# NirajNair/vector-indexer

Hardware: AMD Instinct MI355X
Metric: QPS at recall@10>=0.95 (IVF search, SIFT1M-shaped) (higher is better)
Workload: dtype f32; 1 GPU; IVF search N=1000000 D=128 nlist=4096 nprobe=32 k=10 nq/step=10000 (BASELINE configs[1]); nprobe=32, index_centroids=4094, parallelism=1 GPU

## Files before the change

vector-indexer_amd/csrc/range_select.hip:

```cpp
#include <hip/hip_runtime.h>

#include <algorithm>
#include <cmath>
#include <cstdio>
#include <vector>

#include "select.hpp"
#include "select_device.hpp"

namespace vi {

namespace {

constexpr uint64_t kMaxRangeKeys = 1ull << 27;
constexpr uint32_t kMinRowLog = 11;

struct RangeArgs {
  SelectCommon c;
  uint32_t q0, m, P;
  float radius2;
  ListProbes lp;
  uint32_t *bound;
  uint64_t *keys;
  uint32_t logL;
  uint32_t *counts;
  uint32_t *overflow;
};

__device__ __attribute__((noinline)) float exact_dist_fn(uint32_t form, const float *qrow, const uint32_t *qbytes, uint32_t qn_int,
                                                         const uint4 *x, uint32_t dim, bool live) {
  float d = INFINITY;
  if (live) {
    if (form == 3u) d = exact_pair_u8_int(qbytes, qn_int, x, dim);
    else if (form == 2u) d = exact_pair_u8(qrow, x, dim);
    else if (form == 1u) d = exact_pair_bf16(qrow, x, dim);
    else d = exact_pair<kWave>(qrow, (const float4 *)x, dim);
  }
  return d;
}

template <bool EMIT, bool FILT>
__global__ void __launch_bounds__(256, 4) range_select_kernel(RangeArgs a) {
  __shared__ uint32_t s_pick[4][kPickCap], s_lcache[4][kCacheG];
  __shared__ float4 s_tcache[4][kCacheG];
  __shared__ __attribute__((aligned(16))) uint32_t s_qbytes[4][64];
  extern __shared__ __attribute__((aligned(16))) float s_qrows[];
  const int lane = threadIdx.x & (kWave - 1), wave = threadIdx.x >> 6;
  if (blockIdx.x * 4 + wave >= a.m) return;
  const uint32_t q = a.q0 + blockIdx.x * 4 + wave;
  const SelectCommon &c = a.c;
  uint32_t *pick = s_pick[wave], *qbytes = s_qbytes[wave];
  float *qlds = s_qrows + (size_t)wave * c.dim;
  const ProbeRegs pr = load_probe_regs(a.lp, c.gq, q, a.P, lane);
  const GroupRecords gr{c, a.lp.qoff[q], a.lp.qtot[q], s_tcache[wave], s_lcache[wave]};
  const uint64_t below = (1ull << lane) - 1ull;
  const QueryFrame f = query_frame<EMIT>(c, q, lane, qlds, qbytes);
  float thr = INFINITY;
  if (a.radius2 < 1.0e37f) {
    const float w = ((float)(c.dim >> 6) + 9.0f) * 6.1e-8f * (fabsf(a.radius2) + f.qn);
    thr = rank_threshold(c, f, (a.radius2 - f.qn) + w);
  }
  const uint32_t form = c.u8_nat ? (f.q_bytes ? 3u : 2u) : (c.hi_nat ? 1u : 0u);
  const uint4 *xbase = c.u8_nat ? c.u8_nat : (c.hi_nat ? c.hi_nat : (const uint4 *)c.blocks);
  const uint32_t xmult = c.u8_nat ? c.dq / 4u : (c.hi_nat ? c.dq / 2u : c.dq);
  uint64_t *row = EMIT ? a.keys + ((size_t)(q - a.q0) << a.logL) : nullptr;
  const uint32_t cap = EMIT ? 1u << a.logL : 0u;
  uint32_t npick = 0, n_exact = 0, n_scanned = 0, n_sub = 0, cursor = 0;
  auto exact_emit = [&](bool live, uint32_t r, uint32_t pos) {
    const uint32_t fb = (uint32_t)__shfl((int)pr.fb, (int)r);
    const uint32_t g = (uint32_t)__shfl((int)pr.g, (int)r);
    const uint32_t len = (uint32_t)__shfl((int)pr.len, (int)r);
    live = live && pos < len;
    const uint32_t p = live ? pos : 0u;
    if constexpr (FILT) live = live && ((c.allow[fb + p / kWave] >> (p % kWave)) & 1ull) != 0ull;
    n_exact += (uint32_t)__popcll(__ballot(live));
    const float d = exact_dist_fn(form, qlds, qbytes, f.qn_int, xbase + ((size_t)(fb + p / kWave) * xmult) * kWave + (p % kWave), c.dim, live);
    const bool hit = live && d <= a.radius2;
    const uint64_t m = __ballot(hit);
    if (hit) {
      const uint32_t at = cursor + (uint32_t)__popcll(m & below);
      if (at < cap) row[at] = pack_key(d, (g << kPosBits) | pos);
    }
    cursor += (uint32_t)__popcll(m);
  };
  auto drain = [&]() { drain_pick(c, pick, npick, lane, exact_emit); };
  gr.fill(lane);
  for (uint32_t gb = 0; gb < gr.G; gb += kWave) {
    const uint32_t gidx = gb + lane;
    const bool live = gidx < gr.G;
    uint32_t r, seg, hh;
    gr.group_place(gidx, live, r, seg, hh);
    scan_pair_records(c, pr, lane, live && !(gr.group_values(gidx, live).x > thr), r, seg, hh, n_scanned,
                      [&](bool ok, float v, uint32_t, uint32_t rr, uint32_t sub, uint32_t h2) {
                        const bool want = ok && !(v > thr);
                        if constexpr (EMIT) push_sub(pick, npick, n_sub, lane, want, rr, sub, h2, drain);
                        else n_sub += (uint32_t)__popcll(__ballot(want));
                      });
  }
  if constexpr (EMIT) {
    drain();
    if (lane == 0) {
      a.counts[q] = min(cursor, cap);
      if (cursor > cap) atomicOr(a.overflow, 1u);
    }
    if (c.dbg && lane == 0 && (q & c.dbg_mask) == 0u) {
      atomicAdd(&c.dbg[kStatSelExact], (unsigned long long)n_exact);
      atomicAdd(&c.dbg[kStatSelScanned], (unsigned long long)n_scanned);
      atomicAdd(&c.dbg[kStatSelSubBlocks], (unsigned long long)n_sub);
    }
  } else {
    if (lane == 0) a.bound[q] = 16u * n_sub;
  }
}

struct RangeOutArgs {
  const uint64_t *keys;
  uint32_t logL, q0, m, P;
  const uint32_t *counts, *probes, *gorder, *first_block;
  const uint64_t *lims, *ext_ids;
  float *D;
  int64_t *I;
  uint64_t *tie, *slots;
};

__global__ void __launch_bounds__(256) range_output_kernel(RangeOutArgs a) {
  __shared__ uint32_t s_fb[4][kWave];
  const uint32_t lane = threadIdx.x & (kWave - 1), wave = threadIdx.x >> 6;
  if (blockIdx.x * 4 + wave >= a.m) return;
  const uint32_t q = a.q0 + blockIdx.x * 4 + wave;
  if (lane < a.P) {
    const uint32_t l = a.probes[(size_t)q * a.P + lane], g = a.gorder[(size_t)q * a.P + lane];
    if (l != kNoPos && g < kWave) s_fb[wave][g] = a.first_block[l];
  }
  wave_lds_sync();
  const uint64_t *row = a.keys + ((size_t)(q - a.q0) << a.logL);
  const uint64_t at = a.lims[q];
  const uint32_t n = a.counts[q];
  for (uint32_t i = lane; i < n; i += kWave) {
    const uint64_t key = row[i];
    const uint32_t t = (uint32_t)key, g = t >> kPosBits, pos = t & kPosMask;
    const uint64_t gslot = (uint64_t)s_fb[wave][g & 63u] * kWave + pos;
    a.D[at + i] = sortable_f32((uint32_t)(key >> 32));
    a.I[at + i] = (int64_t)a.ext_ids[gslot];
    a.tie[at + i] = ((uint64_t)g << 32) | pos;
    a.slots[at + i] = gslot;
  }
}

}

vi_status launch_range_select(SearchBatch &b, float radius2, const SelectFrame &f, RangeResult *res) {
  const DeviceIndex &ix = b.ix;
  const EngineKnobs &kn = b.kn;
  SearchWorkspace &ws = b.ws();
  const uint64_t nq = b.nq;
  hipStream_t st = b.st();
  VI_TRY(ws.range_bound.reserve(nq + 1));
  VI_TRY(ws.counts.reserve(nq));
  RangeArgs a{list_select_common(b, f), 0u, (uint32_t)nq, b.P, radius2, list_probes(b), ws.range_bound.p, nullptr, 0u, ws.counts.p,
              ws.range_bound.p + nq};
  if (b.flt) a.c.allow = b.flt->allow.p;
  unsigned long long *dbg = a.c.dbg;
  const size_t qsm = 4ull * ix.dim * sizeof(float);
  hipEvent_t ev[5] = {nullptr, nullptr, nullptr, nullptr, nullptr};
  struct EventGuard { hipEvent_t *e; ~EventGuard() { for (int i = 0; i < 5; ++i) if (e[i]) (void)hipEventDestroy(e[i]); } } guard{ev};
  float ms_step[4] = {0.0f, 0.0f, 0.0f, 0.0f};
  auto mark = [&](int i) -> vi_status {
    if (!kn.stats_print) return VI_OK;
    if (!ev[i]) VI_HIP(hipEventCreate(&ev[i]));
    VI_HIP(hipEventRecord(ev[i], st));
    return VI_OK;
  };
  auto lap = [&](int step, int from, int to) {
    float ms = 0.0f;
    if (kn.stats_print && hipEventElapsedTime(&ms, ev[from], ev[to]) == hipSuccess) ms_step[step] += ms;
  };
  a.c.dbg = nullptr;
  VI_HIP(hipMemsetAsync(ws.range_bound.p + nq, 0, sizeof(uint32_t), st));
  VI_TRY(mark(0));
  hipLaunchKernelGGL((range_select_kernel<false, false>), dim3((uint32_t)((nq + 3) / 4)), dim3(256), qsm, st, a);
  VI_HIP(hipGetLastError());
  VI_TRY(mark(1));
  std::vector<uint32_t> h_bound(nq);
  VI_HIP(hipMemcpyAsync(h_bound.data(), ws.range_bound.p, nq * sizeof(uint32_t), hipMemcpyDeviceToHost, st));
  VI_HIP(hipStreamSynchronize(st));
  lap(0, 0, 1);
  a.c.dbg = dbg;
  uint64_t q0 = 0;
  while (q0 < nq) {
    uint32_t logL = kMinRowLog;
    while ((1ull << logL) < h_bound[q0]) ++logL;
    if ((1ull << logL) > kMaxRangeKeys) return fail(VI_ERR_INVALID_INPUT, "a query's radius admits more candidates than the key scratch holds");
    uint64_t m = 1;
    while (q0 + m < nq) {
      uint32_t lg = logL;
      while ((1ull << lg) < h_bound[q0 + m]) ++lg;
      if ((m + 1) << lg > kMaxRangeKeys) break;
      logL = lg;
      ++m;
    }
    const uint64_t L = 1ull << logL;
    VI_TRY(ws.sort_keys.reserve(m * L));
    VI_TRY(mark(0));
    VI_HIP(hipMemsetAsync(ws.sort_keys.p, 0xFF, m * L * sizeof(uint64_t), st));
    a.q0 = (uint32_t)q0; a.m = (uint32_t)m; a.keys = ws.sort_keys.p; a.logL = logL;
    const dim3 grid((uint32_t)((m + 3) / 4));
    if (b.flt) hipLaunchKernelGGL((range_select_kernel<true, true>), grid, dim3(256), qsm, st, a);
    else hipLaunchKernelGGL((range_select_kernel<true, false>), grid, dim3(256), qsm, st, a);
    VI_HIP(hipGetLastError());
    VI_TRY(mark(1));
    VI_TRY(sort_rows_u64(ws.sort_keys.p, m, logL, st));
    VI_TRY(mark(2));
    VI_TRY(range_result_place(res, q0, m, ws.counts.p + q0, st));
    RangeOutArgs o{ws.sort_keys.p, logL, (uint32_t)q0, (uint32_t)m, b.P, ws.counts.p, ws.probes.p, ws.gorder.p, ix.list_first_block.p,
                   res->lims.p, ix.ext_ids.p, res->D.p, res->I.p, res->tie.p, res->slots.p};
    hipLaunchKernelGGL(range_output_kernel, grid, dim3(256), 0, st, o);
    VI_HIP(hipGetLastError());
    VI_TRY(mark(3));
    if (kn.stats_print) {
      VI_HIP(hipStreamSynchronize(st));
      lap(1, 0, 1); lap(2, 1, 2); lap(3, 2, 3);
    }
    q0 += m;
  }
  uint32_t overflow = 0;
  VI_HIP(hipMemcpyAsync(&overflow, ws.range_bound.p + nq, sizeof(uint32_t), hipMemcpyDeviceToHost, st));
  VI_HIP(hipStreamSynchronize(st));
  if (kn.stats_print) {
    uint64_t bound_total = 0;
    for (uint32_t b : h_bound) bound_total += b;
    fprintf(stderr, "range select ms: bound pass %.4f, evaluation %.4f, sort %.4f, placing + output %.4f; hits %llu of a bound of %llu\n",
            ms_step[0], ms_step[1], ms_step[2], ms_step[3], (unsigned long long)res->total, (unsigned long long)bound_total);
  }
  if (overflow) return fail(VI_ERR_OTHER, "radius select: a query found more hits than its bound pass counted");
  return VI_OK;
}

}
```

vector-indexer_amd/csrc/select.hip:

```cpp
#include "select.hpp"

#include <hip/hip_runtime.h>

#include <cmath>

#include "select_device.hpp"
#include "wave_select.hpp"

namespace vi {
namespace {

template <class Top>
__device__ __attribute__((noinline)) Top offer_bulk_fn(Top s, float dist, uint32_t pos, int K) {
  s.offer_bulk(dist, pos, K);
  return s;
}

template <class Top>
__device__ __attribute__((noinline)) Top exact_batch_fn(Top sel, const float *qrow, const float4 *xv, uint32_t dim, bool live,
                                                        uint32_t key, int K) {
  float d = INFINITY;
  if (live) d = exact_pair<kWave>(qrow, xv, dim);
  sel.offer_bulk(d, live ? key : kNoPos, K);
  return sel;
}

template <class Top>
__device__ __attribute__((noinline)) Top exact_batch_u8_fn(Top sel, const float *qrow, const uint4 *xb, uint32_t dim, bool live, uint32_t key,
                                                           int K) {
  float d = INFINITY;
  if (live) d = exact_pair_u8(qrow, xb, dim);
  sel.offer_bulk(d, live ? key : kNoPos, K);
  return sel;
}

template <class Top>
__device__ __attribute__((noinline)) Top exact_batch_u8_int_fn(Top sel, const uint32_t *qb, uint32_t qn, const uint4 *xb, uint32_t dim, bool live,
                                                               uint32_t key, int K) {
  float d = INFINITY;
  if (live) d = exact_pair_u8_int(qb, qn, xb, dim);
  sel.offer_bulk(d, live ? key : kNoPos, K);
  return sel;
}

template <class Top>
__device__ __attribute__((noinline)) Top exact_batch_row_fn(Top sel, const float *qrow, const float4 *xr, uint32_t dim, bool live,
                                                            uint32_t key, int K) {
  float d = INFINITY;
  if (live) d = exact_pair<1>(qrow, xr, dim);
  sel.offer_bulk(d, live ? key : kNoPos, K);
  return sel;
}

constexpr uint32_t kStageFloats = 2048;
template <class Top>
__device__ __attribute__((noinline)) Top exact_batch_rows_staged_fn(Top sel, const float *qrow, const float4 *rows, uint32_t nrows, uint32_t dim,
                                                                    uint32_t cnt, uint32_t pos, int K, float *stage) {
  const uint32_t lane = threadIdx.x & 63u, r0 = lane >> 2, piece = (lane & 3u) ^ ((lane >> 3) & 3u);
  const uint32_t nquad = dim >> 2, nch = nquad >> 2;
  const VI_AS_LDS vf4 *xq = (const VI_AS_LDS vf4 *)(const VI_AS_LDS float *)qrow;
  const uint32_t sbase = (uint32_t)(size_t)(VI_AS_LDS float *)stage;
  const float4 *src[4];
#pragma unroll
  for (uint32_t j = 0; j < 4; ++j)
    src[j] = rows + (size_t)min((uint32_t)__shfl((int)pos, (int)min(r0 + 16u * j, cnt - 1u)), nrows - 1u) * nquad + piece;
  auto issue = [&](uint32_t c) {
#pragma unroll
    for (uint32_t j = 0; j < 4; ++j) glds16_at(src[j] + 4u * c, sbase + (c & 1u) * 4096u + j * 1024u);
  };
  asm volatile("s_waitcnt vmcnt(0)" ::: "memory");
  issue(0u);
  if (nch > 1u) issue(1u);
  const uint32_t swz = (lane >> 1) & 3u;
  float acc = 0.0f;
#pragma unroll 1
  for (uint32_t c = 0; c < nch; ++c) {
    if (c + 1u < nch) asm volatile("s_waitcnt vmcnt(4)" ::: "memory");
    else asm volatile("s_waitcnt vmcnt(0)" ::: "memory");
    const VI_AS_LDS vf4 *rd = (const VI_AS_LDS vf4 *)((const VI_AS_LDS float *)stage + (c & 1u) * 1024u + lane * 16u);
    const vf4 x0 = rd[0u ^ swz], x1 = rd[1u ^ swz], x2 = rd[2u ^ swz], x3 = rd[3u ^ swz];
    const vf4 q0 = xq[4u * c], q1 = xq[4u * c + 1u], q2 = xq[4u * c + 2u], q3 = xq[4u * c + 3u];
#define VI_PK_QUAD(QQ, XX)                                                         \
  {                                                                                \
    const vf2 ta = pk_sub_f32(QQ.xy, XX.xy), tb = pk_sub_f32(QQ.zw, XX.zw);        \
    const vf2 sa = ta * ta, sb = tb * tb;                                          \
    acc = acc + sa.x; acc = acc + sa.y; acc = acc + sb.x; acc = acc + sb.y;        \
  }
    VI_PK_QUAD(q0, x0) VI_PK_QUAD(q1, x1) VI_PK_QUAD(q2, x2) VI_PK_QUAD(q3, x3)
#undef VI_PK_QUAD
    if (c + 2u < nch) {
      asm volatile("s_waitcnt lgkmcnt(0)" ::: "memory");
      issue(c + 2u);
    }
  }
  const bool live = lane < cnt && pos < nrows;
  sel.offer_bulk(live ? acc : INFINITY, live ? pos : kNoPos, K);
  return sel;
}

template <class Top>
__device__ __attribute__((noinline)) Top exact_batch_bf16_fn(Top sel, const float *qrow, const uint4 *xh, uint32_t dim, bool live,
                                                             uint32_t key, int K) {
  float d = INFINITY;
  if (live) d = exact_pair_bf16(qrow, xh, dim);
  sel.offer_bulk(d, live ? key : kNoPos, K);
  return sel;
}


template <class Top, bool FILT = false>
__device__ __forceinline__ void select_body(const SelectCommon &c, uint32_t q, size_t gbase, uint32_t G, uint32_t P,
                                            const ProbeRegs &pr, uint32_t K, int lane, uint32_t *pick, float4 *tcache,
                                            uint32_t *lcache, float *qlds, Top &sel, uint32_t *qbytes = nullptr) {
  const uint64_t below = (1ull << lane) - 1ull;
  const QueryFrame f = query_frame<true>(c, q, lane, qlds, qbytes);
  uint32_t npick = 0, n_exact = 0, n_scanned = 0, n_full = 0, n_sub = 0;
  Top s1;
  float thr = INFINITY;
  sel.init();
  const float *qrow = qlds;
  auto exact_offer = [&](bool live, uint32_t r, uint32_t pos) {
    const uint32_t fb = (uint32_t)__shfl((int)pr.fb, (int)r);
    const uint32_t g = (uint32_t)__shfl((int)pr.g, (int)r);
    const uint32_t len = (uint32_t)__shfl((int)pr.len, (int)r);
    live = live && pos < len && !(c.xmode & 1u);
    if constexpr (FILT) {
      const uint32_t p = live ? pos : 0u;
      live = live && ((c.allow[fb + p / kWave] >> (p % kWave)) & 1ull) != 0ull;
    }
    n_exact += (uint32_t)__popcll(__ballot(live));
    if (c.u8_nat && f.q_bytes)
      sel = exact_batch_u8_int_fn(sel, qbytes, f.qn_int, c.u8_nat + ((size_t)(fb + (live ? pos : 0u) / kWave) * (c.dq / 4)) * kWave + (pos % kWave),
                                  c.dim, live, (g << kPosBits) | pos, (int)K);
    else if (c.u8_nat)
      sel = exact_batch_u8_fn(sel, qrow, c.u8_nat + ((size_t)(fb + (live ? pos : 0u) / kWave) * (c.dq / 4)) * kWave + (pos % kWave), c.dim,
                              live, (g << kPosBits) | pos, (int)K);
    else if (c.hi_nat)
      sel = exact_batch_bf16_fn(sel, qrow, c.hi_nat + ((size_t)(fb + (live ? pos : 0u) / kWave) * (c.dq / 2)) * kWave + (pos % kWave),
                                c.dim, live, (g << kPosBits) | pos, (int)K);
    else
      sel = exact_batch_fn(sel, qrow, c.blocks + ((size_t)(fb + (live ? pos : 0u) / kWave) * c.dq) * kWave + (pos % kWave),
                           c.dim, live, (g << kPosBits) | pos, (int)K);
  };
  auto drain = [&]() { drain_pick(c, pick, npick, lane, exact_offer); };
  auto scan_groups = [&](bool want, uint32_t r, uint32_t seg, uint32_t hh, int mode) {
    scan_pair_records(c, pr, lane, want, r, seg, hh, n_scanned, [&](bool ok, float v, uint32_t j, uint32_t rr, uint32_t sub, uint32_t h2) {
      if (mode == 0) s1 = offer_bulk_fn(s1, ok ? v : INFINITY, ok ? j : kNoPos, (int)K);
      else push_sub(pick, npick, n_sub, lane, ok && !(v > thr), rr, sub, h2, drain);
    });
  };

  unsigned long long tk = c.dbg ? __builtin_amdgcn_s_memtime() : 0ull, tks[6] = {0, 0, 0, 0, 0, 0};
  auto lap = [&](int i) {
    if (c.dbg) {
      const unsigned long long now = __builtin_amdgcn_s_memtime();
      tks[i] += now - tk;
      tk = now;
    }
  };
  const GroupRecords gr{c, gbase, G, tcache, lcache};
  gr.fill(lane);
  lap(0);
  bool any_full = false;
  {
    s1.init();
    float U = INFINITY;
    if (K <= 64u) {
      float lm = INFINITY;
      for (uint32_t gb = 0; gb < G; gb += kWave) {
        const uint32_t gidx = gb + lane;
        lm = fminf(lm, gr.group_values(gidx, gidx < G).x);
      }
      uint64_t kk = pack_key(lm, (uint32_t)lane);
      wave_sort_u64(kk, lane);
      U = sortable_f32((uint32_t)(readlane_u64(kk, (int)K - 1) >> 32));
    }
    uint32_t ncand = 0;
    bool overflow = !(U < INFINITY);
    if (!overflow) {
      for (uint32_t gb = 0; gb < G && !overflow; gb += kWave) {
        const uint32_t gidx = gb + lane;
        const bool live = gidx < G;
        const float4 T = gr.group_values(gidx, live);
        const float tv[4] = {T.x, T.y, T.z, T.w};
#pragma unroll
        for (uint32_t j = 0; j < 4; ++j) {
          const bool pass = live && !(tv[j] > U);
          const uint64_t m = __ballot(pass);
          if (!m) continue;
          const uint32_t cnt = (uint32_t)__popcll(m);
          if (ncand + cnt > kPickCap / 2u) { overflow = true; break; }
          if (pass) {
            const uint32_t at = ncand + (uint32_t)__popcll(m & below);
            pick[2u * at] = __float_as_uint(tv[j]);
            pick[2u * at + 1u] = 4u * gidx + j;
          }
          ncand += cnt;
        }
      }
      wave_lds_sync();
    }
    if (!overflow) {
      for (uint32_t c0 = 0; c0 < ncand; c0 += kWave) {
        const bool live = c0 + lane < ncand;
        const float v = live ? __uint_as_float(pick[2u * (c0 + lane)]) : INFINITY;
        s1 = offer_bulk_fn(s1, v, live ? pick[2u * (c0 + lane) + 1u] : kNoPos, (int)K);
      }
      wave_lds_sync();
    } else {
      s1.init();
      for (uint32_t gb = 0; gb < G; gb += kWave) {
        const uint32_t gidx = gb + lane;
        const bool live = gidx < G;
        s1 = offer_bulk_fn(s1, gr.group_values(gidx, live).x, live ? 4u * gidx : kNoPos, (int)K);
      }
      for (uint32_t gb = 0; gb < G; gb += kWave) {
        const uint32_t gidx = gb + lane;
        const bool live = gidx < G;
        const float4 T = gr.group_values(gidx, live);
        s1 = offer_bulk_fn(s1, T.y, live ? 4u * gidx + 1u : kNoPos, (int)K);
        s1 = offer_bulk_fn(s1, T.z, live ? 4u * gidx + 2u : kNoPos, (int)K);
        s1 = offer_bulk_fn(s1, T.w, live ? 4u * gidx + 3u : kNoPos, (int)K);
      }
    }
    thr = rank_threshold(c, f, s1.kth((int)K));
    for (uint32_t gb = 0; gb < G; gb += kWave) {
      const uint32_t gidx = gb + lane;
      const float4 T = gr.group_values(gidx, gidx < G);
      any_full = any_full || __ballot(gidx < G && T.w <= thr) != 0ull;
    }
  }
  lap(1);
  if (any_full && !f.distrust && !(c.xmode & 4u)) {
    {
      bool keep[2] = {false, false};
#pragma unroll
      for (int e = 0; e < Top::kEntries; ++e) {
        const uint32_t key = s1.ent_p(e);
        const bool mine = key != kNoPos && (uint32_t)(64 * e + lane) < K;
        keep[e] = mine && !(gr.group_values(mine ? (key >> 2) : 0u, true).w <= thr);
      }
      s1.rebuild(keep[0], keep[1], (int)K);
    }
    for (uint32_t gb = 0; gb < G; gb += kWave) {
      const uint32_t gidx = gb + lane;
      const bool live = gidx < G;
      uint32_t r, seg, hh;
      gr.group_place(gidx, live, r, seg, hh);
      scan_groups(live && gr.group_values(gidx, live).w <= thr, r, seg, hh, 0);
    }
    thr = fminf(thr, rank_threshold(c, f, s1.kth((int)K)));
  }
  lap(2);
  for (uint32_t gb = 0; gb < G; gb += kWave) {
    const uint32_t gidx = gb + lane;
    const bool live = gidx < G;
    uint32_t r, seg, hh;
    gr.group_place(gidx, live, r, seg, hh);
    const float4 T = gr.group_values(gidx, live);
    n_full += (uint32_t)__popcll(__ballot(live && T.w <= thr));
    scan_groups(live && !(T.x > thr) && !(c.xmode & 2u), r, seg, hh, 1);
  }
  lap(3);
  drain();
  lap(4);
  if (c.dbg && lane == 0 && (q & c.dbg_mask) == 0u) {
#pragma unroll
    for (int i = 0; i < 5; ++i) atomicAdd(&c.dbg[kStatClocks + i], tks[i]);
    atomicAdd(&c.dbg[kStatSelExact], (unsigned long long)n_exact);
    atomicAdd(&c.dbg[kStatSelScanned], (unsigned long long)n_scanned);
    atomicAdd(&c.dbg[kStatSelQueriesFull], (unsigned long long)(any_full ? 1u : 0u));
    atomicAdd(&c.dbg[kStatSelFullGroups], (unsigned long long)n_full);
    atomicAdd(&c.dbg[kStatSelSubBlocks], (unsigned long long)n_sub);
  }
}

struct SelectArgs {
  SelectCommon c;
  uint32_t nq, P, k;
  ListProbes lp;
  const uint64_t *ext_ids;
  float *D;
  int64_t *I;
  uint64_t *tie, *slots;
  uint32_t *counts;
};

template <class Top, bool FILT = false>
__global__ void __launch_bounds__(256, 4) select_kernel(SelectArgs a) {
  __shared__ uint32_t s_pick[4][kPickCap], s_lcache[4][kCacheG];
  __shared__ float4 s_tcache[4][kCacheG];
  __shared__ __attribute__((aligned(16))) uint32_t s_qbytes[4][64];
  extern __shared__ __attribute__((aligned(16))) float s_qrows[];
  const int lane = threadIdx.x & (kWave - 1), wave = threadIdx.x >> 6;
  const uint32_t q = blockIdx.x * 4 + wave;
  if (q >= a.nq) return;
  uint32_t mylist;
  const ProbeRegs pr = load_probe_regs(a.lp, a.c.gq, q, a.P, lane, &mylist);
  Top sel;
  select_body<Top, FILT>(a.c, q, a.lp.qoff[q], a.lp.qtot[q], a.P, pr, a.k, lane, s_pick[wave], s_tcache[wave],
                   s_lcache[wave], s_qrows + (size_t)wave * a.c.dim, sel, s_qbytes[wave]);
  uint32_t found = 0;
  const uint32_t inv = (uint32_t)__builtin_amdgcn_ds_permute((int)(4u * (mylist != kNoPos ? pr.g : (uint32_t)lane)), lane);
#pragma unroll
  for (int e = 0; e < Top::kEntries; ++e) {
    const uint32_t key = sel.ent_p(e), idx = 64u * (uint32_t)e + (uint32_t)lane;
    const uint32_t g = key >> kPosBits, pos = key & kPosMask;
    const uint32_t r = (uint32_t)__shfl((int)inv, (int)(g & 63u));
    const bool have = idx < a.k && key != kNoPos;
    found += (uint32_t)__popcll(__ballot(have));
    const uint32_t fbk = (uint32_t)__shfl((int)pr.fb, (int)r);
    if (idx < a.k) {
      const size_t o = (size_t)q * a.k + idx;
      if (have) {
        const uint64_t gslot = (uint64_t)fbk * kWave + pos;
        a.D[o] = sel.ent_d(e);
        a.I[o] = (int64_t)a.ext_ids[gslot];
        if (a.tie) a.tie[o] = ((uint64_t)g << 32) | pos;
        if (a.slots) a.slots[o] = gslot;
      } else {
        a.D[o] = INFINITY;
        a.I[o] = -1;
        if (a.tie) a.tie[o] = ~0ull;
        if (a.slots) a.slots[o] = ~0ull;
      }
    }
  }
  if (a.counts && lane == 0) a.counts[q] = found;
}

struct CoarseSelectArgs {
  SelectCommon c;
  uint32_t nq, P, nlists, segb, recs;
  const uint32_t *list_shard, *list_len;
  uint32_t *probes, *gorder, *cnt;
  const float4 *cent_rows;
  uint32_t list_segb0;
  uint32_t *rel, *qtot;
  uint32_t staged;
  uint32_t *pair_rank;
};

__device__ __forceinline__ void write_probe_row(const CoarseSelectArgs &a, uint32_t q, int lane, uint32_t mylist, uint32_t found,
                                                bool lane_order) {
  const uint32_t g = lane_order ? (uint32_t)lane : probe_candidate_order(lane, found, mylist, a.list_shard);
  if ((uint32_t)lane < a.P) {
    a.probes[(size_t)q * a.P + lane] = mylist;
    a.gorder[(size_t)q * a.P + lane] = g;
    if (mylist != kNoPos && a.list_len[mylist] > 0) {
      const uint32_t before = atomicAdd(&a.cnt[subbin_index(mylist, q & (kSubBins - 1), a.nlists)], 1u);
      if (a.pair_rank) a.pair_rank[(size_t)q * a.P + lane] = before;
    }
  }
  uint32_t ng = 0;
  if (mylist != kNoPos) {
    uint32_t sb;
    ng = 2u * list_segments(a.list_len[mylist], a.list_segb0, &sb);
  }
  const uint32_t ig = wave_incl_scan_u32(ng);
  if ((uint32_t)lane < a.P) a.rel[(size_t)q * a.P + lane] = ig - ng;
  if (lane == 63) a.qtot[q] = ig;
}

__global__ void __launch_bounds__(256, 4) coarse_select_kernel(CoarseSelectArgs a) {
  __shared__ uint32_t s_pick[4][kPickCap], s_lcache[4][kCacheG];
  __shared__ float4 s_tcache[4][kCacheG];
  __shared__ __attribute__((aligned(16))) float s_q[4][kNarrowDim];
  const int lane = threadIdx.x & (kWave - 1), wave = threadIdx.x >> 6;
  const uint32_t q = blockIdx.x * 4 + wave;
  if (q >= a.nq) return;
  ProbeRegs pr{0u, 0u, 0u, 0u, 0u, 1u, 0u};
  if (lane == 0) {
    pr.ng = a.recs; pr.len = a.nlists; pr.segb = a.segb;
    pr.boff = (q / a.c.gq) * (a.recs / 2u) * seg_records(a.segb) * (2u * a.c.gq) + (q % a.c.gq);
  }
  FastTopK sel;
  select_body<FastTopK>(a.c, q, (size_t)q * a.recs, a.recs, 1u, pr, a.P, lane, s_pick[wave], s_tcache[wave],
              s_lcache[wave], s_q[wave], sel);
  const uint32_t found = (uint32_t)__popcll(__ballot((uint32_t)lane < a.P && sel.ent_p(0) != kNoPos));
  const uint32_t mylist = (uint32_t)lane < found ? sel.ent_p(0) : kNoPos;
  write_probe_row(a, q, lane, mylist, found, false);
}

__global__ void __launch_bounds__(256) coarse_select_direct_kernel(CoarseSelectArgs a) {
  __shared__ uint32_t s_pick[4][kPickCap];
  __shared__ __attribute__((aligned(16))) float s_q[4][kNarrowDim];
  __shared__ __attribute__((aligned(16))) float s_stage[4][kStageFloats];
  const int lane = threadIdx.x & (kWave - 1), wave = threadIdx.x >> 6;
  const uint32_t q = blockIdx.x * 4 + wave;
  if (q >= a.nq) return;
  const SelectCommon &c = a.c;
  uint32_t *pick = s_pick[wave];
  float *qlds = s_q[wave];
  const uint64_t below = (1ull << lane) - 1ull;
  unsigned long long tk = c.dbg ? __builtin_amdgcn_s_memtime() : 0ull, tks[6] = {0, 0, 0, 0, 0, 0};
  auto lap = [&](int i) {
    if (c.dbg) {
      const unsigned long long now = __builtin_amdgcn_s_memtime();
      tks[i] += now - tk;
      tk = now;
    }
  };
  const QueryFrame f = query_frame<true>(c, q, lane, qlds, nullptr);
  wave_lds_sync();
  lap(0);
  const uint32_t K = a.P, nblk = (a.nlists + kWave - 1) / kWave, nrec = 4u * nblk;
  constexpr uint32_t kPer = kDirectBlocks * 4 / kWave;
  auto record = [&](uint32_t i) {
    const uint32_t rec = i * kWave + lane;
    float4 r = make_float4(INFINITY, INFINITY, INFINITY, INFINITY);
    if (rec < nrec) r = c.brec[(size_t)q * nrec + rec];
    return r;
  };
  float lm = INFINITY;
// ... 190 lines not shown
```

vector-indexer_amd/csrc/select_device.hpp:

```cpp
#pragma once
#include <hip/hip_runtime.h>

#include <cmath>

#include "device_math.hpp"
#include "mfma_bf16.hpp"
#include "scan.hpp"
#include "search_internal.hpp"
#include "select.hpp"
#include "slot_filter.hpp"
#include "wave_sort.hpp"

namespace vi {

constexpr int kWave = 64;

struct SelectCommon {
  const float *Q;
  uint32_t dim, dq;
  const float4 *blocks;
  const float4 *gval;
  const uint32_t *gmeta;
  const float4 *brec;
  float gamma, e_scale, xmax2;
// ... 158 lines not shown
    for (int i = 0; i < 8; ++i) x[i] = glb_u4(xb + (size_t)(p + i) * kWave);
#pragma unroll
    for (int i = 0; i < 8; ++i) piece(x[i], p + i);
  }
  for (; p < npiece; ++p) piece(glb_u4(xb + (size_t)p * kWave), p);
  return (float)(qn + xx - 2u * dot);
}

__device__ __forceinline__ uint32_t subblock_vector(uint32_t e, uint32_t t, uint32_t hh, bool image_order) {
  return image_order ? 32u * t + 16u * hh + e : 32u * t + (e & 3u) + 8u * (e >> 2) + 4u * hh;
}

constexpr uint32_t kPickCap = 256;
constexpr uint32_t kSubBits = 21;
constexpr uint32_t kCacheG = 256;

struct QueryFrame {
  float qn;
  float E;
  uint32_t qn_int;
  bool q_bytes;
  bool distrust;
};

template <bool STAGE>
__device__ __forceinline__ QueryFrame query_frame(const SelectCommon &c, uint32_t q, int lane, float *qlds, uint32_t *qbytes) {
  QueryFrame f;
  float qn = 0.0f, qres = 0.0f;
  bool q_bytes = c.u8_nat != nullptr && qbytes != nullptr && c.dim <= 256u;
  for (uint32_t e = lane; e < c.dim; e += kWave) {
    const float v = c.Q[(size_t)q * c.dim + e];
    if (STAGE) qlds[e] = v;
    const float vc = c.mu ? v - c.mu[e] : v;
    qn += vc * vc;
    const float im = -2.0f * vc, ir = im - __uint_as_float(bf16_rn(im) << 16);
    qres += ir * ir;
    q_bytes = q_bytes && v >= 0.0f && v <= 255.0f && v == floorf(v);
  }
  f.q_bytes = __ballot(!q_bytes) == 0ull;
#pragma unroll
  for (int o = 32; o > 0; o >>= 1) { qn += __shfl_xor(qn, o); qres += __shfl_xor(qres, o); }
  f.qn = qn;
  f.qn_int = 0u;
  if (STAGE && f.q_bytes) {
    const uint32_t nw = ((c.dim + 15u) >> 4) * 4u;
    for (uint32_t w = lane; w < nw; w += kWave) {
      uint32_t word = 0u;
#pragma unroll
      for (uint32_t b = 0; b < 4; ++b) {
        const uint32_t e = 4u * w + b;
        const uint32_t v = e < c.dim ? (uint32_t)c.Q[(size_t)q * c.dim + e] : 0u;
        word |= v << (8u * b);
        f.qn_int += v * v;
      }
      qbytes[w] = word;
    }
#pragma unroll
    for (int o = 32; o > 0; o >>= 1) f.qn_int += (uint32_t)__shfl_xor((int)f.qn_int, o);
  }
  f.E = c.e_scale * (qn * (1.0f + c.gamma) + 2.0f * c.xmax2) + c.e_abs;
  if (c.trunc) f.E += 1.02f * (2.0f * sqrtf(qn) * c.rho_max * (1.0f + 0.00391f) + (c.trunc == 2u ? sqrtf(qres) * c.vmax : 0.0f));
  f.distrust = !(qn < 1.0e30f);
  return f;
}

__device__ __forceinline__ float rank_threshold(const SelectCommon &c, const QueryFrame &f, float mk) {
  if (f.distrust || !(mk < 1.0e37f)) return INFINITY;
  const float scale = fmaxf(mk + f.qn, 0.0f) + f.E;
  return mk + (2.0f * f.E + 3.0f * c.gamma * scale) * 1.001f + 1e-30f;
}

struct ListProbes {
  const uint32_t *qoff, *qtot, *rel, *pair_pos, *tile_start;
  const uint32_t *probes, *gorder, *first_block, *list_len;
  uint32_t segb0;
};

inline ListProbes list_probes(const SearchBatch &b) {
  const SearchWorkspace &ws = b.ws();
  return ListProbes{ws.qoff.p, ws.qtot.p, ws.pair_rel.p, ws.pair_pos.p, ws.tile_start.p, ws.probes.p, ws.gorder.p,
                    b.ix.list_first_block.p, b.ix.list_len.p, b.kn.segb0};
}

__device__ __forceinline__ ProbeRegs load_probe_regs(const ListProbes &lp, uint32_t gq, uint32_t q, uint32_t P, int lane,
                                                     uint32_t *mylist = nullptr) {
  ProbeRegs pr{0u, 0u, 0u, 0u, 0u, 1u, kNoPos};
  uint32_t list = kNoPos;
  if ((uint32_t)lane < P) {
    const size_t s = (size_t)q * P + lane;
    list = lp.probes[s];
    pr.g = lp.gorder[s];
    pr.rel = lp.rel[s];
    if (list != kNoPos) {
      pr.len = lp.list_len[list];
      pr.fb = lp.first_block[list];
      const uint32_t pp = lp.pair_pos[s];
      const uint32_t nseg = list_segments(pr.len, lp.segb0, &pr.segb);
      pr.ng = 2u * nseg;
      pr.boff = (lp.tile_start[list] + (pp / gq) * nseg * seg_records(pr.segb)) * (2u * gq) + (pp % gq);
    }
  }
  if (mylist) *mylist = list;
  return pr;
}

struct GroupRecords {
  const SelectCommon &c;
  size_t gbase;
  uint32_t G;
  float4 *tcache;
  uint32_t *lcache;

  __device__ __forceinline__ void fill(int lane) const {
    float4 t4[kCacheG / kWave];
#pragma unroll
    for (uint32_t ch = 0; ch < kCacheG / kWave; ++ch) {
      const uint32_t gidx = ch * kWave + lane;
      t4[ch] = make_float4(INFINITY, INFINITY, INFINITY, INFINITY);
      if (gidx < G) t4[ch] = c.gval[gbase + gidx];
    }
    uint32_t l4[kCacheG / kWave];
#pragma unroll
    for (uint32_t ch = 0; ch < kCacheG / kWave; ++ch) {
      const uint32_t gidx = ch * kWave + lane;
      l4[ch] = 0u;
      if (gidx < G) l4[ch] = c.gmeta[gbase + gidx];
    }
#pragma unroll
    for (uint32_t ch = 0; ch < kCacheG / kWave; ++ch) {
      const uint32_t gidx = ch * kWave + lane;
      if (ch * kWave < G) {
        tcache[gidx] = t4[ch];
        lcache[gidx] = l4[ch];
      }
    }
    wave_lds_sync();
  }
  __device__ __forceinline__ float4 group_values(uint32_t gidx, bool live) const {
    float4 T = make_float4(INFINITY, INFINITY, INFINITY, INFINITY);
    if (live) T = gidx < kCacheG ? lds_f4((const float *)(tcache + gidx)) : c.gval[gbase + gidx];
    return T;
  }
  __device__ __forceinline__ void group_place(uint32_t gidx, bool live, uint32_t &r, uint32_t &seg, uint32_t &hh) const {
    uint32_t L = 0u;
    if (live) L = gidx < kCacheG ? *(const VI_AS_LDS uint32_t *)(lcache + gidx) : c.gmeta[gbase + gidx];
    r = L & 63u; seg = (L >> 6) & 127u; hh = L >> 13;
  }
};

template <class Visit>
__device__ __forceinline__ void scan_pair_records(const SelectCommon &c, const ProbeRegs &pr, int lane, bool want, uint32_t r, uint32_t seg,
                                                  uint32_t hh, uint32_t &n_scanned, Visit visit) {
  uint64_t m = __ballot(want);
  const uint32_t slot = (uint32_t)lane >> 4, pi = (uint32_t)lane & 15u;
  while (m) {
    int src = 0;
    uint32_t taken = 0;
#pragma unroll
    for (uint32_t i = 0; i < 4; ++i)
      if (m) {
        const int b = __builtin_ctzll(m);
        m &= m - 1ull;
        if (slot == i) src = b;
        ++taken;
      }
    const bool mine = slot < taken;
    n_scanned += taken;
    const uint32_t rr = (uint32_t)__shfl((int)r, src), sg = (uint32_t)__shfl((int)seg, src);
    const uint32_t h2 = (uint32_t)__shfl((int)hh, src);
    const uint32_t segb = (uint32_t)__shfl((int)pr.segb, (int)rr), ln = (uint32_t)__shfl((int)pr.len, (int)rr);
    const uint32_t boff = (uint32_t)__shfl((int)pr.boff, (int)rr);
    const uint32_t nblk = (ln + kWave - 1) / kWave;
    const uint32_t bs = sg * segb, be = min(nblk, bs + segb);
    const uint32_t ntile = be > bs ? 2u * (be - bs) : 0u;
    const uint32_t npairs = !mine ? 0u : (c.wave_order ? 4u * ((ntile + 15u) / 16u) : (ntile + 3u) / 4u);
    uint32_t mx = npairs;
#pragma unroll
    for (int o = 32; o > 0; o >>= 1) mx = max(mx, (uint32_t)__shfl_xor((int)mx, o));
    for (uint32_t p0 = 0; p0 < mx; p0 += 16u) {
      const uint32_t p = p0 + pi;
      const bool live = p < npairs;
      float4 B = make_float4(INFINITY, INFINITY, INFINITY, INFINITY);
      if (live) B = c.brec[(size_t)boff + 2u * c.gq * (sg * seg_records(segb) + p) + c.gq * h2];
      const float bv[4] = {B.x, B.y, B.z, B.w};
#pragma unroll
      for (uint32_t j = 0; j < 4; ++j) {
        const uint32_t tl = c.wave_order ? 16u * (p >> 2) + 4u * j + (p & 3u) : 4u * p + j;
        const bool ok = live && tl < ntile;
        visit(ok, bv[j], j, rr, 2u * bs + tl, h2);
      }
    }
  }
}

template <class Exact>
__device__ __forceinline__ void drain_pick(const SelectCommon &c, const uint32_t *pick, uint32_t &npick, int lane, Exact exact) {
  while (npick > 0) {
    const uint32_t cnt = npick >= 4u ? 4u : npick;
    npick -= cnt;
    const uint32_t rq = (uint32_t)lane >> 4;
    const bool live = rq < cnt;
    const uint32_t ck = live ? pick[npick + rq] : 0u;
    const uint32_t r = ck >> (kSubBits + 1), sub = (ck >> 1) & ((1u << kSubBits) - 1u), hh = ck & 1u;
    exact(live, r, (sub >> 1) * kWave + subblock_vector((uint32_t)lane & 15u, sub & 1u, hh, c.image_order != 0u));
  }
}

template <class Drain>
__device__ __forceinline__ void push_sub(uint32_t *pick, uint32_t &npick, uint32_t &n_sub, int lane, bool want, uint32_t r, uint32_t sub,
                                         uint32_t hh, Drain drain) {
  const uint64_t m = __ballot(want);
  if (!m) return;
  const uint32_t cnt = (uint32_t)__popcll(m);
  n_sub += cnt;
  if (npick + cnt > kPickCap) drain();
  if (want) pick[npick + (uint32_t)__popcll(m & ((1ull << lane) - 1ull))] = (r << (kSubBits + 1)) | (sub << 1) | hh;
  npick += cnt;
  wave_lds_sync();
}

inline SelectCommon select_common(const SearchBatch &b, const float4 *blocks, float xmax2, uint32_t gq, bool wave_order = false, int trunc = 0) {
  const DeviceIndex &ix = b.ix;
  const EngineKnobs &kn = b.kn;
  const double u = 1.01 * std::ldexp(1.0, -24);
  SelectCommon c{};
  c.Q = b.Qd; c.dim = ix.dim; c.dq = ix.dq; c.blocks = blocks;
  c.gval = (const float4 *)b.ws().gval.p; c.gmeta = (const uint32_t *)b.ws().gpos.p;
  c.brec = (const float4 *)b.ws().brec.p;
  c.gamma = (float)((ix.dim + 2.0) * u);
  const double acc = kn.rank_bf16 ? (3.0 * ix.dim + 2.0) * 2.0 * u + 1.01 * std::ldexp(1.0, -15) : (ix.dim + 2.0) * u;
  const bool centred = ix.centered && kn.rank_bf16;
  c.e_scale = (float)(acc + (centred ? 6.0 * u : 0.0));
  c.e_abs = 0.0f;
  c.trunc = (uint32_t)trunc;
  c.rho_max = (float)(std::sqrt((double)ix.rho2_max) * 1.0001);
  c.vmax = (float)(std::sqrt((double)xmax2) * 1.0001);
  c.xmax2 = xmax2;
  c.mu = centred ? ix.centre.p : nullptr;
  c.gq = gq;
  c.image_order = kn.rank_bf16 ? 1u : 0u;
  c.wave_order = wave_order ? 1u : 0u;
  c.hi_nat = nullptr;
  c.u8_nat = nullptr;
  c.allow = nullptr;
  c.dbg = kn.stats ? (unsigned long long *)b.ws().stats.p : nullptr;
  c.dbg_mask = kn.stats_mask;
  c.xmode = kn.select_xmode;
  return c;
}

inline SelectCommon list_select_common(const SearchBatch &b, const SelectFrame &f) {
  const DeviceIndex &ix = b.ix;
  SelectCommon c = select_common(b, (const float4 *)ix.lists.blocks.p, b.kn.rank_bf16 && ix.centered ? ix.xmax2_c : ix.xmax2, f.gq,
                                 f.wave_order, f.approx);
  if (b.kn.stats_coarse) c.dbg = nullptr;
  c.hi_nat = (const uint4 *)ix.lists_hi_nat.p;
  c.u8_nat = (const uint4 *)ix.lists_u8_nat.p;
  if (f.rank_i8) {
    c.mu = ix.i8_centre.p;
    c.e_scale = 0.0f;
    c.e_abs = 1.0f;
    c.xmax2 = ix.i8_xmax2;
    c.vmax = (float)(std::sqrt((double)ix.i8_xmax2) * 1.0001);
  }
  return c;
}

}
```

Baseline: 27.42 million queries/s.

## Batch sub-block pushes and buffer refine values in IVF select scans

Changes scan_pair_records to precompute per-group tile counts, offsets and keys once, hoist the wave-wide max reduction out of the loop, and hand all four values of a record to the visitor in one call. push_sub4 compacts four ballots into the pick buffer with a single LDS sync instead of one per value. The refine pass now buffers candidate distances in LDS and offers them to the top-k selector in batches, rather than calling offer_bulk for every record value. The aim is fewer wave syncs, fewer shuffles and fewer noinline selector calls, at the cost of extra register pressure and a changed order in which values are offered.

```diff
diff --git a/vector-indexer_amd/csrc/range_select.hip b/vector-indexer_amd/csrc/range_select.hip
--- a/vector-indexer_amd/csrc/range_select.hip
+++ b/vector-indexer_amd/csrc/range_select.hip
@@ -91,10 +91,20 @@
     uint32_t r, seg, hh;
     gr.group_place(gidx, live, r, seg, hh);
     scan_pair_records(c, pr, lane, live && !(gr.group_values(gidx, live).x > thr), r, seg, hh, n_scanned,
-                      [&](bool ok, float v, uint32_t, uint32_t rr, uint32_t sub, uint32_t h2) {
-                        const bool want = ok && !(v > thr);
-                        if constexpr (EMIT) push_sub(pick, npick, n_sub, lane, want, rr, sub, h2, drain);
-                        else n_sub += (uint32_t)__popcll(__ballot(want));
+                      [&](const bool (&ok)[4], const float (&v)[4], const uint32_t (&tl)[4], uint32_t kb) {
+                        bool want[4];
+                        uint32_t key[4];
+#pragma unroll
+                        for (uint32_t j = 0; j < 4; ++j) {
+                          want[j] = ok[j] && !(v[j] > thr);
+                          key[j] = kb + (tl[j] << 1);
+                        }
+                        if constexpr (EMIT) {
+                          push_sub4(pick, npick, n_sub, lane, want, key, drain);
+                        } else {
+#pragma unroll
+                          for (uint32_t j = 0; j < 4; ++j) n_sub += (uint32_t)__popcll(__ballot(want[j]));
+                        }
                       });
   }
   if constexpr (EMIT) {
diff --git a/vector-indexer_amd/csrc/select.hip b/vector-indexer_amd/csrc/select.hip
--- a/vector-indexer_amd/csrc/select.hip
+++ b/vector-indexer_amd/csrc/select.hip
@@ -143,11 +143,40 @@
                            c.dim, live, (g << kPosBits) | pos, (int)K);
   };
   auto drain = [&]() { drain_pick(c, pick, npick, lane, exact_offer); };
-  auto scan_groups = [&](bool want, uint32_t r, uint32_t seg, uint32_t hh, int mode) {
-    scan_pair_records(c, pr, lane, want, r, seg, hh, n_scanned, [&](bool ok, float v, uint32_t j, uint32_t rr, uint32_t sub, uint32_t h2) {
-      if (mode == 0) s1 = offer_bulk_fn(s1, ok ? v : INFINITY, ok ? j : kNoPos, (int)K);
-      else push_sub(pick, npick, n_sub, lane, ok && !(v > thr), rr, sub, h2, drain);
-    });
+  uint32_t nval = 0;
+  auto flush_values = [&]() {
+    for (uint32_t c0 = 0; c0 < nval; c0 += kWave) {
+      const bool live = c0 + lane < nval;
+      s1 = offer_bulk_fn(s1, live ? __uint_as_float(pick[c0 + lane]) : INFINITY, live ? 0u : kNoPos, (int)K);
+    }
+    nval = 0;
+    wave_lds_sync();
+  };
+  auto refine_values = [&](const bool (&ok)[4], const float (&v)[4], const uint32_t (&)[4], uint32_t) {
+    uint64_t m[4];
+#pragma unroll
+    for (uint32_t j = 0; j < 4; ++j) m[j] = __ballot(ok[j] && v[j] <= thr);
+    if (!(m[0] | m[1] | m[2] | m[3])) return;
+    const uint32_t total = (uint32_t)(__popcll(m[0]) + __popcll(m[1]) + __popcll(m[2]) + __popcll(m[3]));
+    if (nval + total > kPickCap) flush_values();
+    uint32_t at = nval;
+#pragma unroll
+    for (uint32_t j = 0; j < 4; ++j) {
+      if (ok[j] && v[j] <= thr) pick[at + (uint32_t)__popcll(m[j] & below)] = __float_as_uint(v[j]);
+      at += (uint32_t)__popcll(m[j]);
+    }
+    nval = at;
+    wave_lds_sync();
+  };
+  auto queue_subs = [&](const bool (&ok)[4], const float (&v)[4], const uint32_t (&tl)[4], uint32_t kb) {
+    bool w[4];
+    uint32_t key[4];
+#pragma unroll
+    for (uint32_t j = 0; j < 4; ++j) {
+      w[j] = ok[j] && !(v[j] > thr);
+      key[j] = kb + (tl[j] << 1);
+    }
+    push_sub4(pick, npick, n_sub, lane, w, key, drain);
   };
 
   unsigned long long tk = c.dbg ? __builtin_amdgcn_s_memtime() : 0ull, tks[6] = {0, 0, 0, 0, 0, 0};
@@ -247,8 +276,9 @@
       const bool live = gidx < G;
       uint32_t r, seg, hh;
       gr.group_place(gidx, live, r, seg, hh);
-      scan_groups(live && gr.group_values(gidx, live).w <= thr, r, seg, hh, 0);
-    }
+      scan_pair_records(c, pr, lane, live && gr.group_values(gidx, live).w <= thr, r, seg, hh, n_scanned, refine_values);
+    }
+    flush_values();
     thr = fminf(thr, rank_threshold(c, f, s1.kth((int)K)));
   }
   lap(2);
@@ -259,7 +289,7 @@
     gr.group_place(gidx, live, r, seg, hh);
     const float4 T = gr.group_values(gidx, live);
     n_full += (uint32_t)__popcll(__ballot(live && T.w <= thr));
-    scan_groups(live && !(T.x > thr) && !(c.xmode & 2u), r, seg, hh, 1);
+    scan_pair_records(c, pr, lane, live && !(T.x > thr) && !(c.xmode & 2u), r, seg, hh, n_scanned, queue_subs);
   }
   lap(3);
   drain();
diff --git a/vector-indexer_amd/csrc/select_device.hpp b/vector-indexer_amd/csrc/select_device.hpp
--- a/vector-indexer_amd/csrc/select_device.hpp
+++ b/vector-indexer_amd/csrc/select_device.hpp
@@ -334,7 +334,25 @@
 __device__ __forceinline__ void scan_pair_records(const SelectCommon &c, const ProbeRegs &pr, int lane, bool want, uint32_t r, uint32_t seg,
                                                   uint32_t hh, uint32_t &n_scanned, Visit visit) {
   uint64_t m = __ballot(want);
+  if (!m) return;
   const uint32_t slot = (uint32_t)lane >> 4, pi = (uint32_t)lane & 15u;
+  uint32_t g_ntile, g_off, g_key;
+  const uint32_t g_boff = (uint32_t)__shfl((int)pr.boff, (int)r);
+  {
+    const uint32_t segb = (uint32_t)__shfl((int)pr.segb, (int)r), ln = (uint32_t)__shfl((int)pr.len, (int)r);
+    const uint32_t nblk = (ln + kWave - 1) / kWave;
+    const uint32_t bs = seg * segb, be = min(nblk, bs + segb);
+    g_ntile = want && be > bs ? 2u * (be - bs) : 0u;
+    g_off = 2u * c.gq * (seg * seg_records(segb)) + c.gq * hh;
+    g_key = (r << (kSubBits + 1)) | ((2u * bs) << 1) | hh;
+  }
+  auto records_of = [&](uint32_t ntile) { return c.wave_order ? 4u * ((ntile + 15u) / 16u) : (ntile + 3u) / 4u; };
+  uint32_t mx = 16u;
+  if (__ballot(records_of(g_ntile) > 16u)) {
+    mx = records_of(g_ntile);
+#pragma unroll
+    for (int o = 32; o > 0; o >>= 1) mx = max(mx, (uint32_t)__shfl_xor((int)mx, o));
+  }
   while (m) {
     int src = 0;
     uint32_t taken = 0;
@@ -348,29 +366,24 @@
       }
     const bool mine = slot < taken;
     n_scanned += taken;
-    const uint32_t rr = (uint32_t)__shfl((int)r, src), sg = (uint32_t)__shfl((int)seg, src);
-    const uint32_t h2 = (uint32_t)__shfl((int)hh, src);
-    const uint32_t segb = (uint32_t)__shfl((int)pr.segb, (int)rr), ln = (uint32_t)__shfl((int)pr.len, (int)rr);
-    const uint32_t boff = (uint32_t)__shfl((int)pr.boff, (int)rr);
-    const uint32_t nblk = (ln + kWave - 1) / kWave;
-    const uint32_t bs = sg * segb, be = min(nblk, bs + segb);
-    const uint32_t ntile = be > bs ? 2u * (be - bs) : 0u;
-    const uint32_t npairs = !mine ? 0u : (c.wave_order ? 4u * ((ntile + 15u) / 16u) : (ntile + 3u) / 4u);
-    uint32_t mx = npairs;
-#pragma unroll
-    for (int o = 32; o > 0; o >>= 1) mx = max(mx, (uint32_t)__shfl_xor((int)mx, o));
+    const uint32_t nt = (uint32_t)__shfl((int)g_ntile, src), off = (uint32_t)__shfl((int)g_off, src);
+    const uint32_t boff = (uint32_t)__shfl((int)g_boff, src), kb = (uint32_t)__shfl((int)g_key, src);
+    const uint32_t ntile = mine ? nt : 0u;
+    const uint32_t npairs = records_of(ntile);
     for (uint32_t p0 = 0; p0 < mx; p0 += 16u) {
       const uint32_t p = p0 + pi;
       const bool live = p < npairs;
       float4 B = make_float4(INFINITY, INFINITY, INFINITY, INFINITY);
-      if (live) B = c.brec[(size_t)boff + 2u * c.gq * (sg * seg_records(segb) + p) + c.gq * h2];
+      if (live) B = c.brec[(size_t)boff + off + 2u * c.gq * p];
       const float bv[4] = {B.x, B.y, B.z, B.w};
+      uint32_t tl[4];
+      bool ok[4];
 #pragma unroll
       for (uint32_t j = 0; j < 4; ++j) {
-        const uint32_t tl = c.wave_order ? 16u * (p >> 2) + 4u * j + (p & 3u) : 4u * p + j;
-        const bool ok = live && tl < ntile;
-        visit(ok, bv[j], j, rr, 2u * bs + tl, h2);
+        tl[j] = c.wave_order ? 16u * (p >> 2) + 4u * j + (p & 3u) : 4u * p + j;
+        ok[j] = live && tl[j] < ntile;
       }
+      visit(ok, bv, tl, kb);
     }
   }
 }
@@ -389,15 +402,23 @@
 }
 
 template <class Drain>
-__device__ __forceinline__ void push_sub(uint32_t *pick, uint32_t &npick, uint32_t &n_sub, int lane, bool want, uint32_t r, uint32_t sub,
-                                         uint32_t hh, Drain drain) {
-  const uint64_t m = __ballot(want);
-  if (!m) return;
-  const uint32_t cnt = (uint32_t)__popcll(m);
-  n_sub += cnt;
-  if (npick + cnt > kPickCap) drain();
-  if (want) pick[npick + (uint32_t)__popcll(m & ((1ull << lane) - 1ull))] = (r << (kSubBits + 1)) | (sub << 1) | hh;
-  npick += cnt;
+__device__ __forceinline__ void push_sub4(uint32_t *pick, uint32_t &npick, uint32_t &n_sub, int lane, const bool (&want)[4],
+                                          const uint32_t (&key)[4], Drain drain) {
+  uint64_t m[4];
+#pragma unroll
+  for (uint32_t j = 0; j < 4; ++j) m[j] = __ballot(want[j]);
+  if (!(m[0] | m[1] | m[2] | m[3])) return;
+  const uint32_t total = (uint32_t)(__popcll(m[0]) + __popcll(m[1]) + __popcll(m[2]) + __popcll(m[3]));
+  n_sub += total;
+  if (npick + total > kPickCap) drain();
+  const uint64_t below = (1ull << lane) - 1ull;
+  uint32_t at = npick;
+#pragma unroll
+  for (uint32_t j = 0; j < 4; ++j) {
+    if (want[j]) pick[at + (uint32_t)__popcll(m[j] & below)] = key[j];
+    at += (uint32_t)__popcll(m[j]);
+  }
+  npick = at;
   wave_lds_sync();
 }
 
```

Result: no change. 27.43 million queries/s (median of 3 runs) (+0.0%).
